# dnjulek/vapoursynth-zip

Hardware: AMD Instinct MI355X
Metric: frames/sec at 4K YUV420P16: Bilateral, BoxBlur, SSIMULACRA2 on 1/2/4/8 MI355X (higher is better)
Workload: dtype u16; 1 GPU; vszip.BoxBlur hradius=vradius=13, 3840x2160 YUV420P16, splitmix64 noise, HBM-resident; parallelism=frame-parallel x1, arena_candidates=3

## Files before the change

vapoursynth-zip_amd/csrc/boxblur_ct.hpp:

```cpp
#pragma once
#include <cmath>
#include <cstdlib>
#include <utility>

#include "plane_table.hpp"

namespace {

#ifndef VSZIP_ST_AUX
#define VSZIP_ST_AUX 2
#endif
#ifndef VSZIP_LD_AUX
#define VSZIP_LD_AUX 0
#endif
#ifndef VSZIP_ST8_AUX
#define VSZIP_ST8_AUX 0
#endif
#ifndef VSZIP_ST16_AUX
#define VSZIP_ST16_AUX 2
#endif
constexpr int kStoreAux = VSZIP_ST_AUX, kLoadAux = VSZIP_LD_AUX, kStoreAux8 = VSZIP_ST8_AUX, kStoreAux16 = VSZIP_ST16_AUX;
typedef uint32_t U32x4 __attribute__((ext_vector_type(4)));
typedef uint32_t U32x2 __attribute__((ext_vector_type(2)));

constexpr int kMaxPlanes = 48;
constexpr int PX = 8;

struct BBPlane {
    const void *src;
    void *dst;
    int sstride, dstride;
    int w, h;
    int block0;
    int ntx;
    int nbands;
    int nperiods;
    int cx0;
};

struct BBParams {
    BBPlane p[kMaxPlanes];
    int nplanes;
    int band_rows;
    int nblocks;
};

constexpr int kRingMaxPlanes = 192;
constexpr int kRingMaxBlocks = 8192;
struct RingParams {
    BBPlane p[kRingMaxPlanes];
    int nplanes;
    int nblocks;
    uint8_t plane_of_block[kRingMaxBlocks];
};

__device__ __forceinline__ int ct_tap_row(int k, int i, int radius, int ih) {
    const int dist_from_bottom = ih - 1 - i;
    if (k < radius) return (i < radius - k) ? min(radius - k - i, ih - 1) : (i - radius + k);
    return (dist_from_bottom < k - radius) ? (i - min(k - radius - dist_from_bottom, i)) : (i - radius + k);
}

template <typename T>
struct Raw8;
template <>
struct Raw8<uint16_t> {
    uint4 q;
};
template <>
struct Raw8<uint8_t> {
    uint2 q;
};

__device__ __forceinline__ void unpack8(const Raw8<uint16_t> &r, uint32_t v[PX]) {
    v[0] = r.q.x & 0xffffu; v[1] = r.q.x >> 16;
    v[2] = r.q.y & 0xffffu; v[3] = r.q.y >> 16;
    v[4] = r.q.z & 0xffffu; v[5] = r.q.z >> 16;
    v[6] = r.q.w & 0xffffu; v[7] = r.q.w >> 16;
}

__device__ __forceinline__ void unpack8(const Raw8<uint8_t> &r, uint32_t v[PX]) {
    v[0] = r.q.x & 0xffu; v[1] = (r.q.x >> 8) & 0xffu; v[2] = (r.q.x >> 16) & 0xffu; v[3] = r.q.x >> 24;
    v[4] = r.q.y & 0xffu; v[5] = (r.q.y >> 8) & 0xffu; v[6] = (r.q.y >> 16) & 0xffu; v[7] = r.q.y >> 24;
}

__device__ __forceinline__ void pack8(const uint32_t v[PX], Raw8<uint16_t> &r) {
    r.q.x = v[0] | (v[1] << 16);
    r.q.y = v[2] | (v[3] << 16);
    r.q.z = v[4] | (v[5] << 16);
    r.q.w = v[6] | (v[7] << 16);
}

__device__ __forceinline__ void pack8(const uint32_t v[PX], Raw8<uint8_t> &r) {
    r.q.x = v[0] | (v[1] << 8) | (v[2] << 16) | (v[3] << 24);
    r.q.y = v[4] | (v[5] << 8) | (v[6] << 16) | (v[7] << 24);
}

template <typename T, int PXN>
struct RawN : Raw8<T> {};
template <>
struct RawN<uint8_t, 16> {
    uint4 q;
};
template <typename T>
__device__ __forceinline__ void unpackN(const RawN<T, 8> &r, uint32_t v[8]) {
    unpack8(static_cast<const Raw8<T> &>(r), v);
}
__device__ __forceinline__ void unpackN(const RawN<uint8_t, 16> &r, uint32_t v[16]) {
    const uint32_t dw[4] = {r.q.x, r.q.y, r.q.z, r.q.w};
#pragma unroll
    for (int k = 0; k < 16; ++k) v[k] = (dw[k >> 2] >> (8 * (k & 3))) & 0xffu;
}

__device__ __forceinline__ int mirror_col(int c, int w) {
    c = c < 0 ? -c - 1 : c;
    c = c >= w ? 2 * w - 1 - c : c;
    return min(max(c, 0), w - 1);
}

template <typename T>
__device__ __forceinline__ Raw8<T> load8(const T *row, int vx0, int w, bool fast) {
    Raw8<T> r;
    if (fast) {
        r.q = *reinterpret_cast<const decltype(r.q) *>(row + vx0);
    } else {
        uint32_t v[PX];
#pragma unroll
        for (int k = 0; k < PX; ++k) v[k] = row[mirror_col(vx0 + k, w)];
        pack8(v, r);
    }
    return r;
}

template <typename T>
__device__ __forceinline__ void store8(T *row, int x0, int w, bool fast, const uint32_t o[PX]);

template <>
__device__ __forceinline__ void store8<uint16_t>(uint16_t *row, int x0, int w, bool fast, const uint32_t o[PX]) {
    if (fast) {
        uint4 q;
        q.x = (o[0] & 0xffffu) | (o[1] << 16);
        q.y = (o[2] & 0xffffu) | (o[3] << 16);
        q.z = (o[4] & 0xffffu) | (o[5] << 16);
        q.w = (o[6] & 0xffffu) | (o[7] << 16);
        *reinterpret_cast<uint4 *>(row + x0) = q;
    } else {
#pragma unroll
        for (int k = 0; k < PX; ++k)
            if (x0 + k < w) row[x0 + k] = (uint16_t)o[k];
    }
}

template <>
__device__ __forceinline__ void store8<uint8_t>(uint8_t *row, int x0, int w, bool fast, const uint32_t o[PX]) {
    if (fast) {
        uint2 q;
        q.x = (o[0] & 0xffu) | ((o[1] & 0xffu) << 8) | ((o[2] & 0xffu) << 16) | (o[3] << 24);
        q.y = (o[4] & 0xffu) | ((o[5] & 0xffu) << 8) | ((o[6] & 0xffu) << 16) | (o[7] << 24);
        *reinterpret_cast<uint2 *>(row + x0) = q;
    } else {
#pragma unroll
        for (int k = 0; k < PX; ++k)
            if (x0 + k < w) row[x0 + k] = (uint8_t)o[k];
    }
}

template <int R>
struct CtGeom {
    static constexpr int K = 2 * R + 1;
    static constexpr int NE = (R + 1 + PX - 1) / PX;
    static constexpr int HL = NE * PX;
    static constexpr int HR = ((R + PX - 1) / PX) * PX;
    static constexpr int OUT_LANES = 64 - NE - HL / PX - HR / PX;
    static constexpr int TWO = OUT_LANES * PX;
};

__device__ __forceinline__ void wave_lds_fence() {
    __builtin_amdgcn_fence(__ATOMIC_RELEASE, "wavefront");
    __builtin_amdgcn_wave_barrier();
    __builtin_amdgcn_fence(__ATOMIC_ACQUIRE, "wavefront");
}

template <typename T, int R, bool DPP>
__global__ __launch_bounds__(64) void boxblur_ct_int_kernel(const BBParams prm) {
    using G = CtGeom<R>;
    constexpr uint32_t K = G::K;
    constexpr uint32_t MAGIC = (uint32_t)(((1ull << 32) + K - 1) / K);
    constexpr uint64_t INV = ((1ull << 32) + R) / K;
    constexpr uint32_t INV2 = (uint32_t)(INV >> 16);
    constexpr uint32_t INVLO = (uint32_t)(INV & 0xffffu);

    __shared__ __attribute__((aligned(16))) uint32_t P[64 * PX];

    const int b = blockIdx.x;
    const BBPlane pl = prm.p[vszip_find_plane(prm, b)];
    const int lb = b - pl.block0;
    const int tx = lb % pl.ntx;
    const int by = lb / pl.ntx;
    const int w = pl.w, h = pl.h;
    const int y0 = by * prm.band_rows;
    const int y1 = min(y0 + prm.band_rows, h);
    const T *src = static_cast<const T *>(pl.src);
    T *dst = static_cast<T *>(pl.dst);

    const int lane = threadIdx.x;
    const int X0 = tx * G::TWO;
    const int vx0 = lane < G::NE ? lane * PX : X0 - G::HL + (lane - G::NE) * PX;
    constexpr int VB = sizeof(T) * PX;
    const bool src_al = ((reinterpret_cast<uintptr_t>(src) | (uintptr_t)((size_t)pl.sstride * sizeof(T))) & (VB - 1)) == 0;
    const bool dst_al = ((reinterpret_cast<uintptr_t>(dst) | (uintptr_t)((size_t)pl.dstride * sizeof(T))) & (VB - 1)) == 0;
    const bool in_fast = src_al && vx0 >= 0 && vx0 + PX <= w;
    const bool is_out = lane >= G::NE + G::HL / PX && lane < G::NE + G::HL / PX + G::OUT_LANES && vx0 < w;
    const bool out_fast = dst_al && vx0 + PX <= w;

    uint32_t col[PX];
#pragma unroll
    for (int k = 0; k < PX; ++k) col[k] = 0;
#pragma unroll 1
    for (int k = 0; k < (int)K; ++k) {
        uint32_t v[PX];
        unpack8(load8<T>(src + (size_t)ct_tap_row(k, y0, R, h) * pl.sstride, vx0, w, in_fast), v);
#pragma unroll
        for (int j = 0; j < PX; ++j) col[j] += v[j];
    }

    const int ci = lane * PX;
#pragma unroll 1
    for (int i = y0; i < y1; ++i) {
        Raw8<T> an, sn;
        const bool more = i + 1 < y1;
        if (more) {
            const int n = i + 1;
            const int ar = (n + R < h) ? n + R : n - 1;
            const int sr = (n <= R) ? R - n + 1 : n - R - 1;
            an = load8<T>(src + (size_t)ar * pl.sstride, vx0, w, in_fast);
            sn = load8<T>(src + (size_t)sr * pl.sstride, vx0, w, in_fast);
        }

        uint32_t p[PX];
#pragma unroll
        for (int k = 0; k < PX; ++k) p[k] = __umulhi(col[k] + R, MAGIC);
#pragma unroll
        for (int k = 1; k < PX; ++k) p[k] += p[k - 1];
        const uint32_t incl = DPP ? wave_incl_scan_dpp(p[PX - 1]) : wave_incl_scan_shfl(p[PX - 1]);
        const uint32_t base = incl - p[PX - 1];
#pragma unroll
        for (int k = 0; k < PX; ++k) p[k] += base;
        *reinterpret_cast<uint4 *>(&P[ci]) = make_uint4(p[0], p[1], p[2], p[3]);
        *reinterpret_cast<uint4 *>(&P[ci + 4]) = make_uint4(p[4], p[5], p[6], p[7]);
        wave_lds_fence();

        if (is_out) {
            const uint32_t e0 = P[R] + P[R - 1];
            const uint32_t krow = 32768u + (uint32_t)(((uint64_t)e0 * INVLO) >> 16);
            uint32_t o[PX];
#pragma unroll
            for (int k = 0; k < PX; ++k) {
                const uint32_t e = P[ci + k + R] - P[ci + k - R - 1];
                o[k] = (uint32_t)(((uint64_t)e * INV2 + krow) >> 16);
            }
            store8<T>(dst + (size_t)i * pl.dstride, vx0, w, out_fast, o);
        }
        wave_lds_fence();

        if (more) {
            uint32_t a[PX], sb[PX];
            unpack8(an, a);
            unpack8(sn, sb);
#pragma unroll
            for (int k = 0; k < PX; ++k) col[k] += a[k] - sb[k];
        }
    }
}



template <int R, int SLOT_VGPRS = 4, int PXN = 8, int RV = R>
struct RingGeom {
    static constexpr int K = 2 * RV + 1;
    static constexpr int HL = ((R + 1 + PXN - 1) / PXN) * PXN;
    static constexpr int HR = ((R + PXN - 1) / PXN) * PXN;
#ifdef VSZIP_RING_OUT_LANES
    static constexpr int OUT_LANES = VSZIP_RING_OUT_LANES < 64 - HL / PXN - HR / PXN ? VSZIP_RING_OUT_LANES : 64 - HL / PXN - HR / PXN;
#else
    static constexpr int OUT_LANES = 64 - HL / PXN - HR / PXN;
#endif
    static constexpr int TWO = OUT_LANES * PXN;
    static constexpr int est_vgprs(int d) { return (2 * RV + 1 + d) * SLOT_VGPRS + (PXN == 16 ? 104 : 56); }
    static constexpr int tier(int v) { return v <= 128 ? 4 : (v <= 168 ? 3 : 2); }
    static constexpr int D3 = (2 * RV + 4) % 3 == 0 ? 3 : ((2 * RV + 6) % 3 == 0 ? 5 : 7);
#ifdef VSZIP_RING_D
    static constexpr int D = VSZIP_RING_D | 1;
    static constexpr int KL = (2 * RV + 1 + D) % 3 == 0 ? 3 : 2;
#else
    static constexpr bool SHALLOW = tier(est_vgprs(1)) > tier(est_vgprs(D3));
    static constexpr int D = SHALLOW ? 1 : D3;
    static constexpr int KL = SHALLOW ? 2 : 3;
#endif
    static constexpr int NR = 2 * RV + 1 + D;
#ifdef VSZIP_RING_WPE
    static constexpr int WPE = VSZIP_RING_WPE;
#else
    static constexpr int WPE = (SLOT_VGPRS == 2 && PXN == 8) ? (tier(est_vgprs(D)) > 3 ? 3 : tier(est_vgprs(D))) : tier(est_vgprs(D));
#endif
    static_assert(NR % KL == 0, "K-column ring must divide the period");
    static constexpr uint32_t MAGIC = K > 1 ? (uint32_t)(((1ull << 32) + K - 1) / K) : 0u;
};

template <typename T, int R, bool GENERAL, int PXN = 8, bool HONLY = false>
struct RingWave {
    static_assert(PXN == 8 || (PXN == 16 && sizeof(T) == 1 && !GENERAL), "16 pixels a lane: 8-bit planes, whole 16-pixel groups");
    static constexpr int RV = HONLY ? 0 : R;
    using G = RingGeom<R, (int)(sizeof(T) * PXN / 4), PXN, RV>;
    using RawT = RawN<T, PXN>;
    using Vec = decltype(RawT{}.q);
    static constexpr int NR = G::NR;
    static constexpr uint64_t INV = ((1ull << 32) + R) / (uint64_t)(2 * R + 1);
    static constexpr uint32_t INV2 = (uint32_t)(INV >> 16);

    RawT ring[NR];
    uint32_t col[PXN];
    uint32_t kcol;
    uint32_t kwgt;
    uint32_t kvo;
    uint32_t kn[G::KL], ko[G::KL];
    uint32_t kn_off, ko_off;
    uint32_t kr_prev;
    uint32_t *P;
    const char *srcb;
    char *dstb;
    uint32_t coff;
    uint32_t doff;
    uint32_t next_off;
    uint32_t out_off;
    uint32_t srow, drow;
    int w, h, lane, c0;
    bool rev, ld_ok, is_out, out_full;
    bool plain;
    __amdgpu_buffer_rsrc_t rs, rd;
    uint32_t sdoff;
    uint32_t psel;
    static constexpr uint32_t kOOB = 0xfffffff0u;

    __device__ __forceinline__ RawT fetch_off(uint32_t row_off) const {
        RawT t;
        if constexpr (sizeof(T) * PXN == 16) {
            const auto v = __builtin_amdgcn_raw_buffer_load_b128(rs, coff, row_off, sizeof(T) == 2 ? kLoadAux : 0);
            t.q = make_uint4(v[0], v[1], v[2], v[3]);
        } else {
            const auto v = __builtin_amdgcn_raw_buffer_load_b64(rs, coff, row_off, 0);
            t.q = make_uint2(v[0], v[1]);
        }
        return t;
    }
    __device__ __forceinline__ uint32_t fetch_px(uint32_t row_off) const {
        if constexpr (sizeof(T) == 2)
            return __builtin_amdgcn_raw_buffer_load_b16(rs, kvo, row_off, 0);
        else
            return __builtin_amdgcn_raw_buffer_load_b8(rs, kvo, row_off, 0);
    }
    __device__ __forceinline__ uint32_t krow_now() const {
        constexpr uint32_t INVLO = (uint32_t)(INV & 0xffffu);
        uint32_t v = __umul24(G::K > 1 ? __umulhi(kcol, G::MAGIC) : kcol, kwgt);
        v += (uint32_t)__builtin_amdgcn_update_dpp(0, (int)v, 0x111, 0xf, 0xf, false);
        v += (uint32_t)__builtin_amdgcn_update_dpp(0, (int)v, 0x112, 0xf, 0xf, false);
        v += (uint32_t)__builtin_amdgcn_update_dpp(0, (int)v, 0x114, 0xf, 0xf, false);
        v += (uint32_t)__builtin_amdgcn_update_dpp(0, (int)v, 0x118, 0xf, 0xf, false);
        uint32_t e0;
        if constexpr (R < 16) {
            e0 = (uint32_t)__builtin_amdgcn_readlane((int)v, 15);
        } else {
            v += (uint32_t)__builtin_amdgcn_update_dpp(0, (int)v, 0x142, 0xa, 0xf, false);
            e0 = (uint32_t)__builtin_amdgcn_readlane((int)v, 31);
        }
        return 32768u + (uint32_t)(((uint64_t)e0 * INVLO) >> 16);
    }

    __device__ __forceinline__ void fix_order(RawT &r) const {
        if constexpr (GENERAL) return;
        if constexpr (sizeof(T) * PXN == 16) {
            const uint4 o = r.q;
            r.q.x = __builtin_amdgcn_perm(o.w, o.x, psel);
            r.q.y = __builtin_amdgcn_perm(o.z, o.y, psel);
            r.q.z = __builtin_amdgcn_perm(o.y, o.z, psel);
            r.q.w = __builtin_amdgcn_perm(o.x, o.w, psel);
        } else {
            const uint2 o = r.q;
            r.q.x = __builtin_amdgcn_perm(o.y, o.x, psel);
            r.q.y = __builtin_amdgcn_perm(o.x, o.y, psel);
        }
    }
    __device__ __forceinline__ uint32_t row_off(int v) const {
        const int r = v < 0 ? -v : (v < h ? v : v - RV - 1);
        return (uint32_t)min(r, h - 1) * srow;
    }

    template <int J>
    __device__ __forceinline__ void fill(int y0) {
        ring[J] = fetch_off(row_off(y0 - RV + J));
    }
    template <int J>
    __device__ __forceinline__ void accum() {
        uint32_t v[PXN];
        fix_order(ring[J]);
        unpackN(ring[J], v);
#pragma unroll
        for (int k = 0; k < PXN; ++k) col[k] += v[k];
    }
    template <int... J>
    __device__ __forceinline__ void fill_all(int y0, std::integer_sequence<int, J...>) {
        (fill<(J + G::K) % NR>(y0), ...);
    }
    template <int... J>
    __device__ __forceinline__ void accum_all(std::integer_sequence<int, J...>) {
        (accum<J>(), ...);
    }

    static __device__ __forceinline__ int pidx(int c) { return (c & (PXN - 1)) * 64 + c / PXN; }

    __device__ __forceinline__ void window_sums(const uint32_t *Pb, uint32_t e[PXN]) const {
        if constexpr (!GENERAL) {
#pragma unroll
            for (int k = 0; k < PXN; ++k) {
                const int hi = k + R, lo = k - R - 1;
                const int hi_px = hi & (PXN - 1), hi_ln = hi / PXN;
                const int lo_px = lo & (PXN - 1), lo_ln = (lo - lo_px) / PXN;
                e[k] = Pb[hi_px * 64 + lane + hi_ln] - Pb[lo_px * 64 + lane + lo_ln];
            }
        } else {
            const int off = lane * PXN - c0;
            auto lds = [&](int idx) { return Pb[pidx(min(max(idx, 0), 64 * PXN - 1))]; };
            const uint32_t qw = lds(w - 1 + off);
#pragma unroll
            for (int k = 0; k < PXN; ++k) {
                const int x = c0 + k;
                const int lo = x - R - 1, ml = R - x - 1;
                uint32_t v = lds(min(x + R, w - 1) + off) + qw - lds(min(2 * w - 2 - x - R, w - 1) + off);
                v -= lo >= 0 ? lds(lo + off) : 0u;
                v += ml >= 0 ? lds(ml + off) : 0u;
                e[k] = v;
            }
        }
    }

    __device__ __forceinline__ void emit_row(const uint32_t e[PXN], uint32_t row_off_bytes, uint32_t kr, bool live) const {
        if constexpr (GENERAL) {
            if (!live || !is_out) return;
        }
        uint32_t t[PXN];
#pragma unroll
        for (int k = 0; k < PXN; ++k) t[k] = __umul24(e[k], INV2) + kr;
        if constexpr (!GENERAL) {
#ifdef VSZIP_DIAG_NO_STORE
            const uint32_t vo = (live && lane == 8) ? sdoff : kOOB;
#else
            const uint32_t vo = live ? sdoff : kOOB;
#endif
            if constexpr (sizeof(T) == 2) {
                U32x4 v;
                v.x = __builtin_amdgcn_perm(t[1], t[0], 0x07060302u);
                v.y = __builtin_amdgcn_perm(t[3], t[2], 0x07060302u);
                v.z = __builtin_amdgcn_perm(t[5], t[4], 0x07060302u);
                v.w = __builtin_amdgcn_perm(t[7], t[6], 0x07060302u);
                __builtin_amdgcn_raw_buffer_store_b128(v, rd, vo, row_off_bytes, kStoreAux);
            } else if constexpr (PXN == 16) {
                uint32_t dw[4];
#pragma unroll
                for (int g = 0; g < 4; ++g) {
                    const uint32_t a0 = __builtin_amdgcn_perm(t[4 * g + 1], t[4 * g], 0x0c0c0602u);
                    const uint32_t a1 = __builtin_amdgcn_perm(t[4 * g + 3], t[4 * g + 2], 0x0c0c0602u);
                    dw[g] = a0 | (a1 << 16);
                }
                U32x4 v;
                v.x = dw[0];
                v.y = dw[1];
                v.z = dw[2];
                v.w = dw[3];
                __builtin_amdgcn_raw_buffer_store_b128(v, rd, vo, row_off_bytes, kStoreAux16);
            } else {
                U32x2 v;
                const uint32_t a0 = __builtin_amdgcn_perm(t[1], t[0], 0x0c0c0602u);
                const uint32_t a1 = __builtin_amdgcn_perm(t[3], t[2], 0x0c0c0602u);
                const uint32_t a2 = __builtin_amdgcn_perm(t[5], t[4], 0x0c0c0602u);
                const uint32_t a3 = __builtin_amdgcn_perm(t[7], t[6], 0x0c0c0602u);
                v.x = a0 | (a1 << 16);
                v.y = a2 | (a3 << 16);
                __builtin_amdgcn_raw_buffer_store_b64(v, rd, vo, row_off_bytes, kStoreAux8);
            }
        } else {
            T *q = reinterpret_cast<T *>(dstb + (row_off_bytes + doff));
            if (out_full) {
                if constexpr (sizeof(T) == 2) {
                    uint4 v;
                    v.x = __builtin_amdgcn_perm(t[1], t[0], 0x07060302u);
                    v.y = __builtin_amdgcn_perm(t[3], t[2], 0x07060302u);
                    v.z = __builtin_amdgcn_perm(t[5], t[4], 0x07060302u);
                    v.w = __builtin_amdgcn_perm(t[7], t[6], 0x07060302u);
                    *reinterpret_cast<uint4 *>(q) = v;
                } else {
                    uint2 v;
                    const uint32_t a0 = __builtin_amdgcn_perm(t[1], t[0], 0x0c0c0602u);
                    const uint32_t a1 = __builtin_amdgcn_perm(t[3], t[2], 0x0c0c0602u);
                    const uint32_t a2 = __builtin_amdgcn_perm(t[5], t[4], 0x0c0c0602u);
                    const uint32_t a3 = __builtin_amdgcn_perm(t[7], t[6], 0x0c0c0602u);
                    v.x = a0 | (a1 << 16);
                    v.y = a2 | (a3 << 16);
                    *reinterpret_cast<uint2 *>(q) = v;
                }
            } else {
#pragma unroll
                for (int k = 0; k < PXN; ++k)
                    if (c0 + k < w) q[k] = (T)(t[k] >> 16);
            }
        }
    }

    template <int S>
    __device__ __forceinline__ void step(int i, int y0) {
        uint32_t *Pa = P + (S & 1) * (64 * PXN);
        const uint32_t *Pb = P + ((S & 1) ^ 1) * (64 * PXN);
        __builtin_amdgcn_sched_barrier(0);

        uint32_t e[PXN];
        const bool have_prev = S > 0 || i > y0;
#ifdef VSZIP_DIAG_NO_HORIZONTAL
#pragma unroll
        for (int k = 0; k < PXN; ++k) e[k] = col[k];
#else
        if (!GENERAL || have_prev) window_sums(Pb, e);
#endif

        uint32_t p[PXN];
#pragma unroll
        for (int k = 0; k < PXN; ++k) {
            if constexpr (G::K == 1) {
                p[k] = col[k];
            } else if constexpr (sizeof(T) == 1) {
                constexpr uint32_t M19 = (uint32_t)(((1u << 19) + G::K - 1) / G::K);
                static_assert((uint64_t)(255u * G::K + RV) * (M19 * G::K - (1u << 19)) < (1u << 19), "8-bit divide-by-k shortcut must be exact");
                p[k] = __umul24(col[k], M19) >> 19;
            } else {
                p[k] = __umulhi(col[k], G::MAGIC);
            }
        }
        if constexpr (GENERAL) {
            const uint32_t m = ld_ok ? 0xffffffffu : 0u;
#pragma unroll
            for (int k = 0; k < PXN; ++k) p[k] &= m;
        }
#ifdef VSZIP_DIAG_NO_HORIZONTAL
        (void)Pa;
        kr_prev += p[0] + p[7];
#else
#pragma unroll
        for (int k = 1; k < PXN; ++k) p[k] += p[k - 1];
        const uint32_t incl = wave_incl_scan_dpp(p[PXN - 1]);
        const uint32_t base = incl - p[PXN - 1];
#pragma unroll
        for (int k = 0; k < PXN; ++k) Pa[k * 64 + lane] = p[k] + base;
#endif

        {
            constexpr int E = (S + 1 + 2 * RV) % NR;
            uint32_t a[PXN], sb[PXN];
            fix_order(ring[E]);
            unpackN(ring[E], a);
            unpackN(ring[S], sb);
#pragma unroll
            for (int k = 0; k < PXN; ++k) col[k] += a[k] - sb[k];
#ifdef VSZIP_DIAG_NO_LOAD
            if (next_off == 0xffffffffu) ring[S] = fetch_off(next_off);
#else
            ring[S] = fetch_off(next_off);
#endif

        }
        const uint32_t kr_cur = krow_now();
        {
            constexpr int J = S % G::KL;
            kcol += kn[J] - ko[J];
#ifndef VSZIP_DIAG_NO_KCOL
            kn[J] = fetch_px(kn_off);
            ko[J] = fetch_px(ko_off);
#endif

        }

        emit_row(e, out_off, kr_prev, have_prev);
        out_off += have_prev ? drow : 0u;
        kr_prev = kr_cur;
        if (plain) {
            next_off += srow;
            kn_off += srow;
            ko_off += srow;
        } else {
            next_off = row_off(i + 2 + RV + G::D);
            kn_off = row_off(i + 2 + RV + G::KL);
            ko_off = row_off(i + 1 - RV + G::KL);
        }
#ifndef VSZIP_DIAG_NO_FENCE
        wave_lds_fence();
#endif
    }

    template <int... S>
    __device__ __forceinline__ void period(int i0, int y0, std::integer_sequence<int, S...>) {
        (step<S>(i0 + S, y0), ...);
    }
};

template <typename T, int R, bool GENERAL, int PXN = 8, bool HONLY = false>
__global__ __launch_bounds__(64, (GENERAL ? 2 : RingGeom<R, (int)(sizeof(T) * PXN / 4), PXN, (HONLY ? 0 : R)>::WPE)) void boxblur_ct_ring_kernel(const RingParams prm) {
    using W = RingWave<T, R, GENERAL, PXN, HONLY>;
    using G = typename W::G;
    constexpr int RV = W::RV;
    static_assert(G::NR % 2 == 0 && G::NR <= 64, "ring period must be even and fit a wave");
    __shared__ __attribute__((aligned(16))) uint32_t P[2 * 64 * PXN];

    const int chunk = (prm.nblocks + 7) >> 3;
    const int b = (int)(blockIdx.x & 7) * chunk + (int)(blockIdx.x >> 3);
    if (b >= prm.nblocks) return;
    const int pi = prm.plane_of_block[b];
    const BBPlane pl = prm.p[pi];
    const int lb = b - pl.block0;
    const int tx = lb % pl.ntx;
    const int by = lb / pl.ntx;
    const int p0 = (int)((long)by * pl.nperiods / pl.nbands);
    const int p1 = (int)((long)(by + 1) * pl.nperiods / pl.nbands);
    const int band_rows = (p1 - p0) * G::NR;
    const int y0 = min(p0 * G::NR, pl.h - band_rows);
    const int w = pl.w;

    W st;
    st.P = P;
    st.w = w;
    st.h = pl.h;
    st.srow = (uint32_t)pl.sstride * (uint32_t)sizeof(T);
    st.drow = (uint32_t)pl.dstride * (uint32_t)sizeof(T);
    st.srcb = static_cast<const char *>(pl.src);
    st.dstb = static_cast<char *>(pl.dst);
    const int lane = threadIdx.x;
    st.lane = lane;
    const int vc0 = pl.cx0 + tx * G::TWO - G::HL + lane * PXN;
    st.c0 = vc0;
    st.is_out = lane >= G::HL / PXN && lane < G::HL / PXN + G::OUT_LANES && vc0 < w;
    st.doff = (uint32_t)(max(vc0, 0) * (int)sizeof(T));
    st.out_full = vc0 + PXN <= w;
    if constexpr (!GENERAL) {
        int g = vc0;
        st.rev = false;
        if (vc0 < 0) {
            g = -vc0 - PXN;
            st.rev = true;
        } else if (vc0 >= w) {
            g = 2 * w - vc0 - PXN;
            st.rev = true;
        }
        g = min(max(g, 0), w - PXN);
        st.coff = (uint32_t)(g * (int)sizeof(T));
        st.ld_ok = true;
    } else {
        st.rev = false;
        st.ld_ok = vc0 >= 0 && vc0 < w;
        st.coff = (uint32_t)(min(max(vc0, 0), ((w - 1) / PXN) * PXN) * (int)sizeof(T));
    }

    st.psel = st.rev ? (sizeof(T) == 2 ? 0x05040706u : 0x04050607u) : 0x03020100u;
    st.sdoff = st.is_out ? st.doff : W::kOOB;
    st.rs = __builtin_amdgcn_make_buffer_rsrc(const_cast<void *>(pl.src), 0, (int)((uint32_t)pl.h * st.srow), 0x00020000);
    st.rd = __builtin_amdgcn_make_buffer_rsrc(pl.dst, 0, (int)((uint32_t)pl.h * st.drow), 0x00020000);
    st.plain = (y0 - RV >= 0) && (y0 + band_rows + RV + G::D + 2 < pl.h);

    st.fill_all(y0, std::make_integer_sequence<int, G::NR>{});
#pragma unroll
    for (int k = 0; k < PXN; ++k) st.col[k] = RV;
    st.accum_all(std::make_integer_sequence<int, (int)G::K>{});
    {
        const int kc = min(lane, R);
        st.kvo = (uint32_t)(kc * (int)sizeof(T));
        st.kwgt = lane < R ? 2u : (lane == R ? 1u : 0u);
        uint32_t acc = RV;
#pragma unroll
        for (int k = 0; k < (int)G::K; ++k) acc += st.fetch_px(st.row_off(y0 - RV + k));
        st.kcol = acc;
#pragma unroll
        for (int j = 0; j < G::KL; ++j) {
            st.kn[j] = st.fetch_px(st.row_off(y0 + j + 1 + RV));
            st.ko[j] = st.fetch_px(st.row_off(y0 + j - RV));
        }
        st.kn_off = st.row_off(y0 + G::KL + 1 + RV);
        st.ko_off = st.row_off(y0 + G::KL - RV);
        st.kr_prev = 0;
    }
    st.next_off = st.row_off(y0 + 1 + RV + G::D);
    st.out_off = (uint32_t)y0 * st.drow;

    const int y1 = y0 + band_rows;
#pragma unroll 1
    for (int i0 = y0; i0 < y1; i0 += G::NR) st.period(i0, y0, std::make_integer_sequence<int, G::NR>{});
    {
        uint32_t e[PXN];
        st.window_sums(P + 64 * PXN, e);
        st.emit_row(e, st.out_off, st.kr_prev, true);
    }
}


template <typename T, int R>
int launch_ct_int(vszip_ctx *ctx, const vszip_plane *planes, int nplanes) {
    using G = CtGeom<R>;
    int done = 0;
    while (done < nplanes) {
        BBParams prm;
        const int n = std::min(kMaxPlanes, nplanes - done);
        prm.nplanes = n;
        long total_px = 0;
        for (int i = 0; i < n; ++i) total_px += (long)planes[done + i].w * planes[done + i].h;
        int band = 64;
        while (band > 16 && total_px / ((long)G::TWO * band) < 4096) band >>= 1;
        prm.band_rows = band;
        int blocks = 0;
        for (int i = 0; i < n; ++i) {
            const vszip_plane &s = planes[done + i];
            BBPlane &d = prm.p[i];
            d.src = s.src;
            d.dst = s.dst;
            d.sstride = (int)s.src_stride;
            d.dstride = (int)s.dst_stride;
            d.w = s.w;
            d.h = s.h;
            d.block0 = blocks;
            d.ntx = (s.w + G::TWO - 1) / G::TWO;
            d.nbands = (s.h + band - 1) / band;
            blocks += d.ntx * d.nbands;
        }
        if (ctx->scan_mode == 1)
            hipLaunchKernelGGL((boxblur_ct_int_kernel<T, R, false>), dim3(blocks), dim3(64), 0, ctx->stream, prm);
        else
            hipLaunchKernelGGL((boxblur_ct_int_kernel<T, R, true>), dim3(blocks), dim3(64), 0, ctx->stream, prm);
        VSZIP_HIP_CHECK(ctx, hipGetLastError());
        done += n;
    }
    return VSZIP_OK;
}

struct RingSpan {
    int cx0, ntx;
};

template <typename T, int R, int PXN, bool HONLY = false>
int ring_plan(const vszip_plane *planes, const RingSpan *spans, int n, double *waves_ret) {
    using G = typename RingWave<T, R, false, PXN, HONLY>::G;
    struct Geo {
        int h, ntx, count;
    };
    std::vector<Geo> geos;
    for (int i = 0; i < n; ++i) {
        bool found = false;
        for (Geo &g : geos)
            if (g.h == planes[i].h && g.ntx == spans[i].ntx) {
                ++g.count;
                found = true;
                break;
            }
        if (!found) geos.push_back({planes[i].h, spans[i].ntx, 1});
    }
        auto bands_for = [](int h, int P, int target) { return std::max((h % G::NR != 0 && P >= 2) ? 2 : 1, (P + target / 2) / target); };
        const double halo_p = (double)(G::K - 1 + G::D) / G::NR;
        const double slots = 256.0 * 4 * G::WPE;
        double waves_out = 0;
        auto cost_for = [&](int target) {
            double work = 0, waves = 0, max_len = 0;
            for (const Geo &g : geos) {
                const int P = (g.h + G::NR - 1) / G::NR;
                const int nb = bands_for(g.h, P, target);
                const double ntx = (double)g.ntx * g.count;
                work += ntx * (P + nb * halo_p);
                waves += ntx * nb;
                max_len = std::max(max_len, (double)((P + nb - 1) / nb) + halo_p);
            }
            waves_out = waves;
            const double gens = std::ceil(waves / slots);
            const double eff = std::min(1.0, work / (slots * gens * max_len));
            return std::max(work / slots * (1.0 + 0.3 * (1.0 - eff)), 0.3 * max_len);
        };
        int target = 1;
        double best = cost_for(1);
        const double min_waves = std::min(0.6 * slots, waves_out);
        for (int t = 2; t <= 96; ++t) {
            const double c = cost_for(t);
            if (waves_out >= min_waves && c < best) {
                best = c;
                target = t;
            }
        }
        *waves_ret = (cost_for(target), waves_out);
        return target;
}


template <typename T, int R, int PXN, bool GEN, bool HONLY = false>
int launch_ct_ring_spans(vszip_ctx *ctx, const vszip_plane *all_planes, const RingSpan *all_spans, int nall) {
    using G = typename RingWave<T, R, false, PXN, HONLY>::G;
    std::vector<vszip_plane> planes_v;
    std::vector<RingSpan> spans_v;
    for (int i = 0; i < nall; ++i)
        if (all_spans[i].ntx > 0) {
            planes_v.push_back(all_planes[i]);
            spans_v.push_back(all_spans[i]);
        }
    const vszip_plane *planes = planes_v.data();
    const RingSpan *spans = spans_v.data();
    const int nplanes = (int)planes_v.size();
    int done = 0;
    while (done < nplanes) {
        RingParams prm;
        const int n = std::min(kRingMaxPlanes, nplanes - done);
        auto bands_for = [](int h, int P, int target) { return std::max((h % G::NR != 0 && P >= 2) ? 2 : 1, (P + target / 2) / target); };
        double waves_out = 0;
        int target = ring_plan<T, R, PXN, HONLY>(planes + done, spans + done, n, &waves_out);
        if (ctx->opt.ring_periods > 0) target = ctx->opt.ring_periods;
#ifdef VSZIP_RING_PERIODS_FIXED
        target = VSZIP_RING_PERIODS_FIXED;
#endif
#ifdef VSZIP_RING_PLAN_DEBUG
        fprintf(stderr, "ring plan PX%d GEN%d r=%d: n=%d target=%d waves=%.0f slots=%d NR=%d | plane0 %dx%d ntx=%d\n", PXN, (int)GEN, R, n, target, waves_out, 256 * 4 * G::WPE, G::NR,
                planes[done].w, planes[done].h, spans[done].ntx);
#endif
        VSZIP_HIP_CHECK(ctx, hipSetDevice(ctx->device));
        int blocks = 0, fit = n;
        for (int i = 0; i < n; ++i) {
            const vszip_plane &s = planes[done + i];
            BBPlane &d = prm.p[i];
            d.src = s.src;
            d.dst = s.dst;
            d.sstride = (int)s.src_stride;
            d.dstride = (int)s.dst_stride;
            d.w = s.w;
            d.h = s.h;
            d.nperiods = (s.h + G::NR - 1) / G::NR;
            d.nbands = bands_for(s.h, d.nperiods, target);
            d.ntx = spans[done + i].ntx;
            d.cx0 = spans[done + i].cx0;
            d.block0 = blocks;
            if (blocks + d.ntx * d.nbands > kRingMaxBlocks) {
                if (i == 0) return vszip_set_error(ctx, VSZIP_ERR_ARG, "BoxBlur: launch table overflow (%d blocks)", blocks + d.ntx * d.nbands);
                fit = i;
                break;
            }
            for (int k = 0; k < d.ntx * d.nbands; ++k) prm.plane_of_block[blocks + k] = (uint8_t)i;
            blocks += d.ntx * d.nbands;
        }
        prm.nplanes = fit;
        prm.nblocks = blocks;
        const dim3 grid(((blocks + 7) / 8) * 8);
        {
            vszip_probe_scope probe(ctx);
            hipLaunchKernelGGL((boxblur_ct_ring_kernel<T, R, GEN, PXN, HONLY>), grid, dim3(64), 0, ctx->stream, prm);
        }
        VSZIP_HIP_CHECK(ctx, hipGetLastError());
        done += fit;
    }
    return VSZIP_OK;
}

template <typename T>
bool ring_ok(const vszip_plane *planes, int nplanes) {
    constexpr uintptr_t VB = sizeof(T) * PX;
    for (int i = 0; i < nplanes; ++i) {
        const vszip_plane &p = planes[i];
        if ((reinterpret_cast<uintptr_t>(p.src) | reinterpret_cast<uintptr_t>(p.dst) | (uintptr_t)(p.src_stride * sizeof(T)) | (uintptr_t)(p.dst_stride * sizeof(T))) & (VB - 1)) return false;
        if (p.src_stride < ((p.w + PX - 1) / PX) * PX) return false;
        if (p.src_stride < 24) return false;
        if (p.h < 2 * 22 + 1 + 8) return false;
        if ((uint64_t)p.src_stride * p.h * sizeof(T) >= (1ull << 32) || (uint64_t)p.dst_stride * p.h * sizeof(T) >= (1ull << 32)) return false;
    }
    return true;
}

constexpr int kRing16MaxR = 19;
template <typename T, int R, bool HONLY = false>
bool ring16_ok(const vszip_ctx *ctx, const vszip_plane *planes, int nplanes) {
    if (sizeof(T) != 1 || ctx->opt.ct_u8_px8) return false;
    using G16 = RingGeom<R, 4, 16, (HONLY ? 0 : R)>;
    using G8 = RingGeom<R, 2, 8, (HONLY ? 0 : R)>;
    double px = 0, t16 = 0, t8 = 0;
    for (int i = 0; i < nplanes; ++i) {
        const vszip_plane &p = planes[i];
        if (p.w < 32) return false;
        if ((reinterpret_cast<uintptr_t>(p.src) | reinterpret_cast<uintptr_t>(p.dst) | (uintptr_t)p.src_stride | (uintptr_t)p.dst_stride) & 15) return false;
        px += (double)p.w * p.h;
        t16 += (double)((p.w + G16::TWO - 1) / G16::TWO) * G16::TWO * p.h;
        t8 += (double)((p.w + G8::TWO - 1) / G8::TWO) * G8::TWO * p.h;
    }
    if (R >= 8 && px / t16 < 0.93 * (px / t8)) return false;
    if (R >= 8) {
        const int n = std::min(nplanes, kRingMaxPlanes);
        std::vector<RingSpan> s16(n), s8(n);
        for (int i = 0; i < n; ++i) {
            s16[i] = {0, (planes[i].w + G16::TWO - 1) / G16::TWO};
            s8[i] = {0, (planes[i].w + G8::TWO - 1) / G8::TWO};
        }
        double w16 = 0, w8 = 0;
        ring_plan<T, R, 16, HONLY>(planes, s16.data(), n, &w16);
        ring_plan<T, R, 8, HONLY>(planes, s8.data(), n, &w8);
        const double f16 = w16 / (256.0 * 4 * G16::WPE), f8 = w8 / (256.0 * 4 * G8::WPE);
        if (f16 < 0.8 && f8 > f16 + 0.05) return false;
    }
    return true;
}

template <typename T, int R, int PXF, bool HONLY = false>
int run_ct_ring(vszip_ctx *ctx, const vszip_plane *planes, int nplanes) {
    using GF = typename RingWave<T, R, false, PXF, HONLY>::G;
    using GG = typename RingWave<T, R, true, 8, HONLY>::G;
    std::vector<RingSpan> fast(nplanes), rest(nplanes);
    bool any_rest = false, any_fast = false;
    for (int i = 0; i < nplanes; ++i) {
        const int w = planes[i].w;
        if (w % PXF == 0) {
            fast[i] = {0, (w + GF::TWO - 1) / GF::TWO};
            rest[i] = {0, 0};
        } else {
            const int room = w + GF::HL - 64 * PXF;
            const int nsafe = room >= 0 ? room / GF::TWO + 1 : 0;
            fast[i] = {0, nsafe};
            const int x = nsafe * GF::TWO;
            rest[i] = {x, (w - x + GG::TWO - 1) / GG::TWO};
        }
        any_fast = any_fast || fast[i].ntx > 0;
        any_rest = any_rest || rest[i].ntx > 0;
    }
    if (any_fast) {
        const int rc = launch_ct_ring_spans<T, R, PXF, false, HONLY>(ctx, planes, fast.data(), nplanes);
        if (rc != VSZIP_OK) return rc;
    }
    if (any_rest) return launch_ct_ring_spans<T, R, 8, true, HONLY>(ctx, planes, rest.data(), nplanes);
    return VSZIP_OK;
}

#ifdef VSZIP_DEV_R
#define VSZIP_R_ENABLED(R) ((R) == VSZIP_DEV_R)
#else
#define VSZIP_R_ENABLED(R) true
#endif

template <typename T, int R, int RLO>
struct CtIntDispatch {
    static int run(vszip_ctx *ctx, int r, const vszip_plane *planes, int nplanes) {
        if constexpr (VSZIP_R_ENABLED(R)) if (r == R) {
            if (ctx->scan_mode == 0 && ring_ok<T>(planes, nplanes)) {
                if constexpr (sizeof(T) == 1 && R <= kRing16MaxR) {
                    if (ring16_ok<T, R>(ctx, planes, nplanes)) return run_ct_ring<T, R, 16>(ctx, planes, nplanes);
                }
                return run_ct_ring<T, R, 8>(ctx, planes, nplanes);
            }
            return launch_ct_int<T, R>(ctx, planes, nplanes);
        }
        if constexpr (R > RLO)
            return CtIntDispatch<T, R - 1, RLO>::run(ctx, r, planes, nplanes);
        else
            return vszip_set_error(ctx, VSZIP_ERR_ARG, "BoxBlur: CT radius not built (development build?)");
    }
    static int run_h(vszip_ctx *ctx, int r, const vszip_plane *planes, int nplanes) {
        if constexpr (VSZIP_R_ENABLED(R)) if (r == R) {
            if (ctx->scan_mode != 0 || !ring_ok<T>(planes, nplanes)) return VSZIP_ERR_UNSUPPORTED;
            if constexpr (sizeof(T) == 1) {
                if (ring16_ok<T, R, true>(ctx, planes, nplanes)) return run_ct_ring<T, R, 16, true>(ctx, planes, nplanes);
            }
            return run_ct_ring<T, R, 8, true>(ctx, planes, nplanes);
        }
        if constexpr (R > RLO)
            return CtIntDispatch<T, R - 1, RLO>::run_h(ctx, r, planes, nplanes);
        else
            return VSZIP_ERR_UNSUPPORTED;
    }
};

}
```

Baseline: 111,900 frames/s.

## Split ring BoxBlur bands at row granularity instead of whole periods

Introduces row-granular band splitting for the ring BoxBlur kernel. Bands no longer have to be multiples of the ring period, and the last band need not overlap earlier ones. The per-period loop can now exit early at the band end and selects the right LDS half for the final row. The planner searches band counts under a row-based cost model, with a floor on wave count. The aim is to cut redundant overlap work and balance bands better across CUs, at the cost of an extra per-step exit compare and different scheduling for the configurations that keep period bands.

```diff
diff --git a/vapoursynth-zip_amd/csrc/boxblur_ct.hpp b/vapoursynth-zip_amd/csrc/boxblur_ct.hpp
--- a/vapoursynth-zip_amd/csrc/boxblur_ct.hpp
+++ b/vapoursynth-zip_amd/csrc/boxblur_ct.hpp
@@ -1,4 +1,5 @@
 #pragma once
+#include <climits>
 #include <cmath>
 #include <cstdlib>
 #include <utility>
@@ -34,9 +35,24 @@
     int block0;
     int ntx;
     int nbands;
-    int nperiods;
     int cx0;
 };
+
+constexpr int kRingMaxBands = 32768;
+__host__ __device__ __forceinline__ int ring_band_begin(int by, int h, int nb) {
+    const uint32_t q = (uint32_t)h / (uint32_t)nb, rem = (uint32_t)h - q * (uint32_t)nb;
+    return (int)((uint32_t)by * q + (uint32_t)by * rem / (uint32_t)nb);
+}
+__host__ __device__ __forceinline__ int ring_band_rows(bool row_bands, int NR, int by, int h, int nb, int *y0) {
+    if (row_bands) {
+        *y0 = ring_band_begin(by, h, nb);
+        return ring_band_begin(by + 1, h, nb) - *y0;
+    }
+    const int nperiods = (h + NR - 1) / NR, p0 = ring_band_begin(by, nperiods, nb);
+    const int rows = (ring_band_begin(by + 1, nperiods, nb) - p0) * NR;
+    *y0 = p0 * NR < h - rows ? p0 * NR : h - rows;
+    return rows;
+}
 
 struct BBParams {
     BBPlane p[kMaxPlanes];
@@ -314,6 +330,7 @@
     using RawT = RawN<T, PXN>;
     using Vec = decltype(RawT{}.q);
     static constexpr int NR = G::NR;
+    static constexpr bool ROW_BANDS = !(sizeof(T) == 2 && PXN == 8 && !HONLY && (GENERAL ? R >= 14 : ((R >= 5 && R <= 7) || R == 21)));
     static constexpr uint64_t INV = ((1ull << 32) + R) / (uint64_t)(2 * R + 1);
     static constexpr uint32_t INV2 = (uint32_t)(INV >> 16);
 
@@ -603,7 +620,11 @@
     }
 
     template <int... S>
-    __device__ __forceinline__ void period(int i0, int y0, std::integer_sequence<int, S...>) {
+    __device__ __forceinline__ bool period(int i0, int y0, int y1, std::integer_sequence<int, S...>) {
+        return ((step<S>(i0 + S, y0), i0 + S + 1 == y1) || ...);
+    }
+    template <int... S>
+    __device__ __forceinline__ void whole_period(int i0, int y0, std::integer_sequence<int, S...>) {
         (step<S>(i0 + S, y0), ...);
     }
 };
@@ -624,10 +645,8 @@
     const int lb = b - pl.block0;
     const int tx = lb % pl.ntx;
     const int by = lb / pl.ntx;
-    const int p0 = (int)((long)by * pl.nperiods / pl.nbands);
-    const int p1 = (int)((long)(by + 1) * pl.nperiods / pl.nbands);
-    const int band_rows = (p1 - p0) * G::NR;
-    const int y0 = min(p0 * G::NR, pl.h - band_rows);
+    int y0;
+    const int band_rows = ring_band_rows(W::ROW_BANDS, G::NR, by, pl.h, pl.nbands, &y0);
     const int w = pl.w;
 
     W st;
@@ -694,12 +713,24 @@
     st.next_off = st.row_off(y0 + 1 + RV + G::D);
     st.out_off = (uint32_t)y0 * st.drow;
 
-    const int y1 = y0 + band_rows;
+    uint32_t e[PXN];
+    if constexpr (W::ROW_BANDS) {
+        if (band_rows <= 0) return;
+        const int y1 = __builtin_amdgcn_readfirstlane(y0 + band_rows);
 #pragma unroll 1
-    for (int i0 = y0; i0 < y1; i0 += G::NR) st.period(i0, y0, std::make_integer_sequence<int, G::NR>{});
+        for (int i0 = y0;; i0 += G::NR)
+            if (st.period(i0, y0, y1, std::make_integer_sequence<int, G::NR>{})) break;
+        if (__builtin_amdgcn_readfirstlane(band_rows) & 1)
+            st.window_sums(P, e);
+        else
+            st.window_sums(P + 64 * PXN, e);
+    } else {
+        const int y1 = y0 + band_rows;
+#pragma unroll 1
+        for (int i0 = y0; i0 < y1; i0 += G::NR) st.whole_period(i0, y0, std::make_integer_sequence<int, G::NR>{});
+        st.window_sums(P + 64 * PXN, e);
+    }
     {
-        uint32_t e[PXN];
-        st.window_sums(P + 64 * PXN, e);
         st.emit_row(e, st.out_off, st.kr_prev, true);
     }
 }
@@ -747,8 +778,13 @@
     int cx0, ntx;
 };
 
+inline int ring_bands_for(int h, int NR, int target, bool row_bands) {
+    const int P = (h + NR - 1) / NR, nb = (P + target / 2) / target;
+    return std::min(kRingMaxBands, row_bands ? std::max(1, std::min(h / NR, nb)) : std::max(h % NR != 0 && P >= 2 ? 2 : 1, nb));
+}
+
 template <typename T, int R, int PXN, bool HONLY = false>
-int ring_plan(const vszip_plane *planes, const RingSpan *spans, int n, double *waves_ret) {
+int ring_plan(const vszip_plane *planes, const RingSpan *spans, int n, double *waves_ret, bool row_bands = true) {
     using G = typename RingWave<T, R, false, PXN, HONLY>::G;
     struct Geo {
         int h, ntx, count;
@@ -764,36 +800,42 @@
             }
         if (!found) geos.push_back({planes[i].h, spans[i].ntx, 1});
     }
-        auto bands_for = [](int h, int P, int target) { return std::max((h % G::NR != 0 && P >= 2) ? 2 : 1, (P + target / 2) / target); };
-        const double halo_p = (double)(G::K - 1 + G::D) / G::NR;
+        const double halo = (double)(G::K - 1 + G::D);
         const double slots = 256.0 * 4 * G::WPE;
         double waves_out = 0;
-        auto cost_for = [&](int target) {
+        auto cost_for = [&](int target, bool whole_periods = false) {
             double work = 0, waves = 0, max_len = 0;
             for (const Geo &g : geos) {
-                const int P = (g.h + G::NR - 1) / G::NR;
-                const int nb = bands_for(g.h, P, target);
+                const int nb = ring_bands_for(g.h, G::NR, target, row_bands && !whole_periods);
+                const int rows = whole_periods ? (g.h + G::NR - 1) / G::NR * G::NR : g.h, unit = whole_periods ? G::NR : 1;
                 const double ntx = (double)g.ntx * g.count;
-                work += ntx * (P + nb * halo_p);
+                work += ntx * (rows + nb * halo);
                 waves += ntx * nb;
-                max_len = std::max(max_len, (double)((P + nb - 1) / nb) + halo_p);
+                max_len = std::max(max_len, (double)((rows / unit + nb - 1) / nb * unit) + halo);
             }
             waves_out = waves;
             const double gens = std::ceil(waves / slots);
             const double eff = std::min(1.0, work / (slots * gens * max_len));
             return std::max(work / slots * (1.0 + 0.3 * (1.0 - eff)), 0.3 * max_len);
         };
-        int target = 1;
-        double best = cost_for(1);
-        const double min_waves = std::min(0.6 * slots, waves_out);
-        for (int t = 2; t <= 96; ++t) {
-            const double c = cost_for(t);
-            if (waves_out >= min_waves && c < best) {
-                best = c;
-                target = t;
-            }
-        }
-        *waves_ret = (cost_for(target), waves_out);
+        auto search = [&](bool whole_periods, double floor_waves) {
+            int target = 1;
+            double best = cost_for(1, whole_periods);
+            const double min_waves = std::max(floor_waves, std::min(0.6 * slots, waves_out));
+            for (int t = 2; t <= 96; ++t) {
+                const double c = cost_for(t, whole_periods);
+                if (waves_out >= min_waves && c < best) {
+                    best = c;
+                    target = t;
+                }
+            }
+            return target;
+        };
+        const int t_whole = search(true, 0.0);
+        cost_for(t_whole, true);
+        const double floor_waves = waves_out >= 0.6 * slots ? waves_out : 0.0;
+        const int target = row_bands ? search(false, floor_waves) : t_whole;
+        *waves_ret = (cost_for(target, !row_bands), waves_out);
         return target;
 }
 
@@ -815,9 +857,9 @@
     while (done < nplanes) {
         RingParams prm;
         const int n = std::min(kRingMaxPlanes, nplanes - done);
-        auto bands_for = [](int h, int P, int target) { return std::max((h % G::NR != 0 && P >= 2) ? 2 : 1, (P + target / 2) / target); };
+        constexpr bool kRowBands = RingWave<T, R, GEN, PXN, HONLY>::ROW_BANDS;
         double waves_out = 0;
-        int target = ring_plan<T, R, PXN, HONLY>(planes + done, spans + done, n, &waves_out);
+        int target = ring_plan<T, R, PXN, HONLY>(planes + done, spans + done, n, &waves_out, kRowBands);
         if (ctx->opt.ring_periods > 0) target = ctx->opt.ring_periods;
 #ifdef VSZIP_RING_PERIODS_FIXED
         target = VSZIP_RING_PERIODS_FIXED;
@@ -837,8 +879,7 @@
             d.dstride = (int)s.dst_stride;
             d.w = s.w;
             d.h = s.h;
-            d.nperiods = (s.h + G::NR - 1) / G::NR;
-            d.nbands = bands_for(s.h, d.nperiods, target);
+            d.nbands = ring_bands_for(s.h, G::NR, target, kRowBands);
             d.ntx = spans[done + i].ntx;
             d.cx0 = spans[done + i].cx0;
             d.block0 = blocks;
@@ -852,6 +893,15 @@
         }
         prm.nplanes = fit;
         prm.nblocks = blocks;
+#ifdef VSZIP_RING_PLAN_DEBUG
+        for (int i = 0; i < fit; ++i) {
+            const BBPlane &d = prm.p[i];
+            if (i > 0 && d.h == prm.p[i - 1].h && d.nbands == prm.p[i - 1].nbands) continue;
+            int y0;
+            const int first = ring_band_rows(kRowBands, G::NR, 0, d.h, d.nbands, &y0), last = ring_band_rows(kRowBands, G::NR, d.nbands - 1, d.h, d.nbands, &y0);
+            fprintf(stderr, "ring plan   plane %d: h=%d nb=%d row_bands=%d first band %d rows, last band rows [%d, %d)\n", i, d.h, d.nbands, (int)kRowBands, first, y0, y0 + last);
+        }
+#endif
         const dim3 grid(((blocks + 7) / 8) * 8);
         {
             vszip_probe_scope probe(ctx);
```

Result: no change. 112,700 frames/s (median of 3 runs) (+0.8%).
